# cyberlife-coder/velesdb

Measured on AMD Instinct MI355X. Metric: qps_at_recall10_1Mx768_k10, higher is better.
Workload: dtype f32; 1 GPU; 1000000x768 f32 cosine, k=10, exact distance sweep + fused GPU top-k (BASELINE configs[1]); 1024 queries/step, 1024 queries per corpus pass (sweep_topk_gemm_bf16_pp<dot, WIDE> over normalised bf16 images of rows and queries (cosine; ping-po; rows=1000000, dim=768, k=10, parallelism=replicas x1 (query stream split, no collective)

## Files before the change

velesdb_amd/csrc/g16_protocol.inc:

```
#ifndef VDB_PP_STAMP_AT
#define VDB_PP_STAMP_AT(SLOT) do { } while (0)
#define VDB_G16_OWN_STAMP_STUB 1
#endif
#ifndef VDB_PP_STAMP_COUNT
#define VDB_PP_STAMP_COUNT(SLOT) do { } while (0)
#define VDB_PP_STAMP_ADD(SLOT, N) do { } while (0)
#endif
    VDB_PP_STAMP_AT(16);
    if (hm[0] | hm[1] | hm[2] | hm[3]) VDB_PP_STAMP_COUNT(19);
    VDB_PP_STAMP_ADD(22, __popcll(hm[0]) + __popcll(hm[1]) + __popcll(hm[2]) + __popcll(hm[3]));
    for (;;) {
      ++epoch;
      VDB_PP_STAMP_COUNT(23);
      bool pend = false;
      {
        const uint32_t ln1 = lane_now();
        uint32_t fill = qcnt;
        uint32_t hsz = 64u;
        bool stop = false;
#define VDB_G16_SCAN(T) \
        while (hm[T] && !stop) { \
          if (hsz == 1u && fill + 32u > (uint32_t)QCAP) {  \
            stop = true; \
            break; \
          } \
          const uint32_t hrank = __builtin_amdgcn_mbcnt_hi((uint32_t)(hm[T] >> 32), __builtin_amdgcn_mbcnt_lo((uint32_t)hm[T], 0u)); \
          const bool mine = (((hm[T] >> ln1) & 1ull) != 0) & (hrank < hsz); \
          const uint64_t msk = __ballot(mine); \
          uint32_t nf = fill; \
          const uint32_t hi0 = ((uint32_t)(wr * 128) + 4u * (ln1 >> 4)) | (((uint32_t)(wq * 64 + (T) * 16) + (ln1 & 15u)) << 8); \
_Pragma("unroll") \
          for (int g8 = 0; g8 < 4; g8++) { \
            if (!__ballot(mine & (((gmv[T] >> g8) & 1u) != 0u))) continue;  \
_Pragma("unroll") \
            for (int j8 = 0; j8 < 8; j8++) { \
// ... 20 lines not shown
            if (lanes == 1u) {  \
              stop = true; \
              break; \
            } \
            continue; \
          } \
          fill = nf; \
          hm[T] &= ~msk; \
        }
#define VDB_G16_FINISH(HAVE, RAW, FITS) do { \
          const uint64_t raw_ = (RAW); \
          const uint32_t b = (uint32_t)(raw_ >> 40) & 255u; \
          const float x = __uint_as_float((uint32_t)raw_); \
          const uint32_t rl = (uint32_t)(raw_ >> 32) & 255u; \
          const uint32_t row = rt * BM + rl; \
          float score; \
          if (METRIC == kHamming) {   \
            score = 0.5f * (qn[b] - x); \
          } else if (METRIC == kJaccard) {   \
            const float uni = qn[b] + vns[rl] - x; \
            score = uni == 0.0f ? 1.0f : x / uni; \
          } else { \
            score = halfp ? finish_score_half<METRIC>(x, qn[b], METRIC == kCosine ? vns[rl] : 1.0f) \
                          : finish_score<METRIC>(x, qn[b], METRIC == kCosine ? vns[rl] : 1.0f); \
          } \
           \
          if constexpr (WIDE) score = canon_nan(score); \
          const uint64_t key = make_key<HIB>(score, row); \
          bool take = (HAVE) & (row < a.n_rows) & (key < tauk[b]); \
          if (take && a.alive) take = a.alive[row] != 0;   \
          if constexpr (WIDE) { \
             \
            if (take) { \
              const uint32_t si = atomicAdd(&cnts[b], 1u); \
              if (si < (uint32_t)CAP) { \
                cand[(size_t)b * CAP + si] = key; \
              } else { \
                const uint32_t qg = q0 + b; \
                const uint32_t gi = atomicAdd(&a.wide_cnt[qg], 1u); \
                if (gi < a.wide_cap) a.wide_keys[(size_t)qg * a.wide_cap + gi] = key; \
              } \
            } \
            FITS = true; \
          } else { \
          const uint64_t mt = __ballot(take); \
          FITS = qcnt + (uint32_t)__popcll(mt) <= (uint32_t)QCAP; \
          if (FITS) { \
            if (take) { \
              const uint32_t slot = qcnt + __builtin_amdgcn_mbcnt_hi((uint32_t)(mt >> 32), __builtin_amdgcn_mbcnt_lo((uint32_t)mt, 0u)); \
              wq_keys[slot] = key; \
              wq_qs[slot] = (uint8_t)b; \
            } \
            qcnt += (uint32_t)__popcll(mt); \
          } \
          } \
        } while (0)
#ifndef VDB_G16_NO_DUMP
        if ((uint32_t)__popcll(hm[0]) + (uint32_t)__popcll(hm[1]) + (uint32_t)__popcll(hm[2]) + (uint32_t)__popcll(hm[3]) <= (uint32_t)kG16DumpMaxLanes) {
          bool dump_ok = true;
          if (hm[0] | hm[1] | hm[2] | hm[3]) VDB_PP_STAMP_COUNT(21);
          float* dump = reinterpret_cast<float*>(wq_keys + 8);
#define VDB_G16_DUMP(T) \
          while (hm[T] && dump_ok) { \
            if (qcnt > 8u) { \
              dump_ok = false; \
              break; \
            } \
            VDB_PP_STAMP_COUNT(24);  \
            const uint32_t h0 = (uint32_t)__builtin_ctzll(hm[T]); \
// ... 37 lines not shown
          if (hm[3]) VDB_G16_MASKS(3);
#undef VDB_G16_MASKS
          gm_lazy = false;
        }
        for (;;) {
          VDB_G16_SCAN(0)
          VDB_G16_SCAN(1)
          VDB_G16_SCAN(2)
          VDB_G16_SCAN(3)
          VDB_PP_STAMP_AT(17);
          if (fill > qcnt) {
            const bool have = ln1 < fill - qcnt;
            const uint64_t raw = have ? wq_keys[qcnt + ln1] : 0ull;
            bool fits;
            VDB_G16_FINISH(have, raw, fits);
            (void)fits;
            fill = qcnt;
            VDB_PP_STAMP_AT(18);
          }
          if (!stop) break;
          if (qcnt + 32u > (uint32_t)QCAP) {
            pend = true;
            break;
          }
          stop = false;
        }
#undef VDB_G16_SCAN
#undef VDB_G16_FINISH
      }
      VDB_PP_STAMP_AT(12);
      if constexpr (WIDE) {
        __syncthreads();
        VDB_PP_STAMP_AT(13);
        break;
      }
      if (pend || (last && qcnt)) flags[0] = epoch;
      __syncthreads();
      VDB_PP_STAMP_AT(13);
      if constexpr (!WIDE) {
      if (flags[1] == epoch) {
        compact();
        __syncthreads();
        VDB_PP_STAMP_AT(14);
      }
      }
      bool want = false;
      {
        const uint32_t ln3 = lane_now();
        const uint64_t key = ln3 < qcnt ? wq_keys[ln3] : kKeyInvalid;
        const uint32_t b = ln3 < qcnt ? wq_qs[ln3] : 0u;
        bool full = false;
        if (key != kKeyInvalid && key < tauk[b]) {
          const uint32_t idx = atomicAdd(&cnts[b], 1u);
          if (idx < (uint32_t)CAP) {
            cand[(size_t)b * CAP + idx] = key;
            want = idx >= k;
          } else {
            full = true;
            want = true;
          }
        }
        const uint64_t mf = __ballot(full);
        qcnt = (uint32_t)__popcll(mf);
        if (full) {
          const uint32_t slot = __builtin_amdgcn_mbcnt_hi((uint32_t)(mf >> 32), __builtin_amdgcn_mbcnt_lo((uint32_t)mf, 0u));
          wq_keys[slot] = key;
          wq_qs[slot] = (uint8_t)b;
        }
      }
      if (__ballot(want)) flags[1] = epoch + 1;
      VDB_PP_STAMP_AT(15);
      bool again = flags[0] >= epoch;
      if (last) {
        if (qcnt) flags[2] = epoch;
        __syncthreads();
        again |= flags[2] == epoch;
      }
      if (!again) break;
    }
#ifdef VDB_G16_OWN_STAMP_STUB
#undef VDB_PP_STAMP_AT
#undef VDB_G16_OWN_STAMP_STUB
#endif
```

velesdb_amd/csrc/g16_writeout.inc:

```
  if constexpr (WIDE) {
  __syncthreads();
  uint32_t* wbase = reinterpret_cast<uint32_t*>(qn);
  const uint32_t t_o = (uint32_t)wib * 64u + lane_now();
  if (t_o < nq_t) {
    const uint32_t n = min(cnts[t_o], (uint32_t)CAP);
    wbase[t_o] = n ? atomicAdd(&a.wide_cnt[q0 + t_o], n) : 0u;
  }
  __syncthreads();
  for (uint32_t i = t_o; i < nq_t * (uint32_t)CAP; i += (uint32_t)WAVES * 64u) {
    const uint32_t b = i / (uint32_t)CAP, e = i - b * (uint32_t)CAP;
    const uint32_t pos = wbase[b] + e;
    if (e < cnts[b] && pos < a.wide_cap) a.wide_keys[(size_t)(q0 + b) * a.wide_cap + pos] = cand[i];
  }
  }
  if constexpr (!WIDE) {
  __syncthreads();
  compact();
  __syncthreads();
  const uint32_t lane_o = lane_now();
  for (uint32_t b = wib; b < nq_t; b += WAVES) {
    const uint32_t c = min(cnts[b], k);
    uint64_t* out = a.part_keys + ((size_t)(q0 + b) * a.list_stride + a.list_off + g) * k;
    for (uint32_t e = lane_o; e < k; e += 64) out[e] = e < c ? cand[(size_t)b * CAP + e] : kKeyInvalid;
    if (a.blk_tau && lane_o == 0) a.blk_tau[(size_t)(q0 + b) * a.list_stride + a.list_off + g] = tauk[b];
  }
  }
```

velesdb_amd/csrc/select_stage.hip:

```cpp
#include <algorithm>
#include <array>
#include <cstdio>
#include <cstdlib>
#include <cstring>
#include <string>
#include <vector>

#include "vdb_probe_env.hpp"
#include "vdb_select_stage.hpp"
#include "vdb_wide.hpp"

namespace vdb {

static inline uint32_t opt_max_tile(const vdb_hip_index* ix) { return (uint32_t)opt_value(ix, VDB_OPT_MAX_QUERY_TILE); }
static inline int opt_engine(const vdb_hip_index* ix) { return (int)opt_value(ix, VDB_OPT_SWEEP_ENGINE); }
static inline int opt_selector(const vdb_hip_index* ix) { return (int)opt_value(ix, VDB_OPT_SELECTOR_LEVEL); }
static const bool g_bf16_seed = [] {
  const char* e = probe_env("VELESDB_BF16_SEED");
  return !(e && e[0] == '0');
}();
static const bool g_pool_select = [] {
  const char* e = probe_env("VELESDB_POOL_SELECT");
  return !(e && e[0] == '0');
}();
// ... 786 lines not shown
        mf.skip_cnt = qcount;
        mf.skip_le = kFallbackGatherMax;
      }
      launch_merge(true, mf, nqg, st);
      fin.fb_ids = mf.out_ids;
      fin.fb_scores = mf.out_scores;
      fin.fb_n = mf.out_n;
    }
    if (gather_ok) {
      fin.max_listed = gather_all ? 0u : kFallbackGatherMax;
      fin.g_ids = mg.out_ids;
      fin.g_scores = mg.out_scores;
      fin.g_n = mg.out_n;
    }
    launch_select_finish(fin, st);
  }
  ix->split_flags_off = o_flags;
  ix->split_flags_n = nqg;
  ix->split_flags_stream = st;
  if (ev) (void)hipEventRecord(ev->b, st);
  VDB_HIP(hipGetLastError());
  return VDB_OK;
}


static const bool g_wide_small_k = [] {
  const char* e = probe_env("VELESDB_WIDE_SMALL_K");
  return !(e && e[0] == '0');
}();
static const bool g_wide_fuse = [] {
  const char* e = probe_env("VELESDB_WIDE_FUSE");
  return !(e && e[0] == '0');
}();
int select_level_wide(vdb_hip_index* ix, uint32_t nq_left, uint32_t k, bool sq8) {
  if (opt_selector(ix) < 2 || (!sq8 && opt_engine(ix) != 1) || opt_max_tile(ix) < 128) return 0;
  if (ix->metric != VDB_COSINE && ix->metric != VDB_DOT && (sq8 || ix->metric != VDB_EUCLIDEAN)) return 0;
  if (ix->dim % 64 != 0 || ix->dim < 128 || ix->row_stride != ix->dim) return 0;
  if (k == 0 || k > kWideMaxK || ix->n_rows < kGemmBf16MinRows || ix->n_rows >= 0xFFFFFF00ull) return 0;
  if (k <= kGemmBf16MaxK && (opt_selector(ix) < 3 || !g_wide_small_k)) return 0;
  if (!sq8 && ix->metric != VDB_EUCLIDEAN && sweep_mfma_lds_bytes(1, k, ix->dim) > 160 * 1024) return 0;
  if (!sq8 && ix->metric == VDB_EUCLIDEAN && !l2_gather_fits(ix->dim, k)) return 0;
  if (!select_chunk(nq_left, sq8 ? kSelectMinQueriesSq8 : 0)) return 0;
  if (ix->sel_stats && ix->sel_stats[2] != ix->sel_seq_seen) {
    ix->sel_seq_seen = ix->sel_stats[2];
    if (ix->sel_stats[3] == 4u && (uint64_t)ix->sel_stats[0] * 16 > ix->sel_stats[1]) ix->wide_hold = 64;
  }
  if (ix->wide_hold) {
    ix->wide_hold--;
    return 0;
  }
  return 4;
}

int32_t brute_wide_dev(vdb_hip_index* ix, const float* d_q, uint64_t q_stride, uint32_t nqg, uint32_t k, uint64_t* d_ids, float* d_scores,
                       uint32_t* d_n, hipStream_t st, bool sq8) {
  const bool cosn = !sq8 && cosine_normalised(ix);
  const bool l2 = !sq8 && ix->metric == VDB_EUCLIDEAN;
  const int sel_metric = (cosn || l2) ? VDB_DOT : ix->metric;
  int32_t rc = sq8 ? ensure_sq8_select(ix, st) : (l2 ? ensure_l2_select(ix, st) : (cosn ? ensure_cosn(ix, st) : ensure_sel16(ix, st)));
  if (rc != VDB_OK) return rc;
  const uint32_t dim_a = ix->dim + 64, dim_s = ix->dim + 4;
  const uint16_t* img_rows = sq8 ? ix->sq8_img.as<uint16_t>()
                                 : (l2 ? ix->l2_img.as<uint16_t>() : (cosn ? ix->cosn_img.as<uint16_t>() : ix->rows_bf16.as<uint16_t>()));
  const uint64_t img_stride = l2 ? (uint64_t)dim_a : ((cosn || sq8) ? (uint64_t)ix->dim : ix->bf16_stride);
  const DevBuf& rho_buf = sq8 ? ix->sq8_rho : (l2 ? ix->l2_rho : (cosn ? ix->cosn_rho : ix->bf16_rho));
  const float* sel_norms = sq8 ? ix->sq8_nrm.as<float>() : ix->norms.as<float>();
  DevBuf& list_buf = sq8 ? ix->s_part_cnt : ix->s_fb_keys;
  const uint32_t sel_dim = l2 ? dim_a : ix->dim;
  ix->last_select_level = 4;
  ix->last_kernels |= VDB_KERNEL_SELECT_BF16;
  const uint8_t* alive = ix->any_dead ? ix->alive.as<uint8_t>() : nullptr;
  const uint32_t n = (uint32_t)ix->n_rows, dim = ix->dim;
  static const uint32_t g_small_seed_rows = [] {
    const char* e = probe_env("VELESDB_WIDE_SEED_ROWS");
    const long v = e ? atol(e) : 0;
    return v >= 1024 && v <= (long)kWideSeedRows ? (uint32_t)v / 256u * 256u : kSplitSeedRows;
  }();
  const uint32_t R0 = std::min<uint32_t>(k <= kWideSmallSeedMaxK ? g_small_seed_rows : kWideSeedRows, n), ngrp = (R0 + 15) / 16;
  GemmSchedule sch;
  {
    static const std::array<uint32_t, 3> mult = [] {
      std::array<uint32_t, 3> m{1, 4, 16};
      if (const char* e = probe_env("VELESDB_WIDE_STEPS")) {
        unsigned a = 0, b = 0, c = 0;
        const int got = sscanf(e, "%u,%u,%u", &a, &b, &c);
        m = {got >= 1 ? a : 0u, got >= 2 ? b : 0u, got >= 3 ? c : 0u};
      }
      return m;
    }();
    const uint32_t head[3] = {mult[0], mult[1], mult[2]};
    gemm_schedule(nqg, 0, n, ix->n_cus, head, 0, &sch);
  }
  int g_nqt = 3;
  while (g_nqt > 1 && sweep_mfma_lds_bytes(g_nqt, k, dim) > 160 * 1024) g_nqt--;
  const int g_waves = g_nqt >= 2 ? kMfmaWaves2 : kMfmaWaves1;
  const uint32_t g_B = l2 ? 8u : (uint32_t)g_nqt * 16;
  const uint32_t ntiles16 = (n + 15) / 16;
  const int g_blocks = l2 ? blocks_for(ix, 8, (n + 7) / 8)
                          : (int)std::max<int64_t>(1, std::min<int64_t>(((int64_t)ntiles16 + g_waves - 1) / g_waves, (int64_t)ix->n_cus));
  size_t off = 0;
  auto take = [&](size_t bytes) {
    const size_t o = off;
    off = (off + bytes + 15) & ~(size_t)15;
    return o;
  };
  const size_t o_tau = take((size_t)nqg * 8), o_delta = take((size_t)nqg * 4), o_qn = take((size_t)nqg * 4), o_rho = take((size_t)nqg * 4),
               o_cnt = take((size_t)nqg * 4), o_state = take((size_t)nqg * 4), o_flags = take((size_t)nqg * 4 + 16), o_qmap = take((size_t)nqg * 8),
               o_gid = take((size_t)nqg * k * 8), o_gsc = take((size_t)nqg * k * 4), o_gn = take((size_t)nqg * 4), o_nmax = take(16),
               o_extra = take((size_t)nqg * 4);
  hipError_t e;
  if ((e = ix->s_seed.reserve(off, false, st)) != hipSuccess || (e = list_buf.reserve((size_t)nqg * kWideCap * 8, false, st)) != hipSuccess ||
      (e = ix->s_part_keys.reserve((size_t)nqg * ngrp * 8, false, st)) != hipSuccess ||
      (!sq8 && (e = ix->s_part_cnt.reserve((size_t)nqg * g_blocks * k * 8, false, st)) != hipSuccess) ||
      (e = ix->s_misc.reserve(((size_t)nqg + 256) * img_stride * 2 + (l2 ? (size_t)nqg * dim_s * 4 + 16 : 0), false, st)) != hipSuccess)
    return fail(VDB_ERR_OOM, "wide selection scratch");
  unsigned char* sd = ix->s_seed.as<unsigned char>();
  uint16_t* q16 = ix->s_misc.as<uint16_t>();
  float* qnorms = reinterpret_cast<float*>(sd + o_qn);
  float* rho_q = rho_buf.p ? reinterpret_cast<float*>(sd + o_rho) : nullptr;
  uint32_t* flags = reinterpret_cast<uint32_t*>(sd + o_flags);
  uint32_t* qcount = flags + nqg;
  uint32_t* qmap = reinterpret_cast<uint32_t*>(sd + o_qmap);
  uint32_t* qslot = qmap + nqg;
  uint32_t* norm_max = reinterpret_cast<uint32_t*>(sd + o_nmax);
  EventPair* ev = next_events(ix);
  if (ev) (void)hipEventRecord(ev->a, st);
  if (l2) {
    float* qaug = reinterpret_cast<float*>(ix->s_misc.as<unsigned char>() + ((((size_t)nqg + 256) * img_stride * 2 + 15) & ~(size_t)15));
    launch_l2_augment_queries(d_q, q_stride, q16, dim_a, qaug, dim_s, nqg, dim, st);
    if (rho_q) launch_query_round_error(d_q, q_stride, rho_q, nqg, dim, st);
    PrepArgs pq{};
    pq.rows = d_q;
    pq.norms = qnorms;
    pq.row_stride = q_stride;
    pq.n_rows = nqg;
    pq.dim = dim;
    pq.words = ix->words;
    launch_prep_rows(pq, st);
    VDB_HIP(hipMemsetAsync(flags, 0, (size_t)nqg * 4 + 16, st));
  } else if (cosn) launch_seln_prep_queries(d_q, q_stride, q16, img_stride, qnorms, rho_q, flags, nqg + 4, nqg, dim, st);
  else launch_sel16_prep_queries(d_q, q_stride, q16, img_stride, qnorms, rho_q, flags, nqg + 4, nqg, dim, st);
  if (nqg % 256u) VDB_HIP(hipMemsetAsync(q16 + (size_t)nqg * img_stride, 0, (size_t)256 * img_stride * 2, st));
  if (ix->metric == VDB_DOT || l2) launch_max_norm(sel_norms, n, norm_max, st);
  WideArgs wa{};
  wa.keys = list_buf.as<uint64_t>();
  wa.eps_extra = sq8 ? 1.5e-4f : 0.0f;
  wa.cnt = reinterpret_cast<uint32_t*>(sd + o_cnt);
  wa.state = reinterpret_cast<uint32_t*>(sd + o_state);
  wa.tau = reinterpret_cast<uint64_t*>(sd + o_tau);
  wa.delta = reinterpret_cast<float*>(sd + o_delta);
  wa.qnorms = qnorms;
  wa.rho_q = rho_q;
  wa.rho_max_bits = rho_q ? rho_buf.as<uint32_t>() : nullptr;
  wa.norm_max_bits = norm_max;
  wa.extra = l2 ? reinterpret_cast<float*>(sd + o_extra) : nullptr;
  wa.cap = kWideCap;
  wa.k = k;
  wa.dim = dim;
  launch_seed_scores_bf16(sel_metric, img_rows, img_stride, sel_norms, alive, q16, img_stride, qnorms, ix->s_part_keys.as<uint64_t>(), R0,
                          nqg, sel_dim, st);
  if (l2) launch_wide_seed_l2(wa, ix->s_part_keys.as<uint64_t>(), ngrp, dim_a, nqg, st);
  else launch_wide_seed(ix->metric, wa, ix->s_part_keys.as<uint64_t>(), ngrp, nqg, st);
  for (int j = 0; j < sch.n_launch; j++) {
    EventPair* evs = next_sel_events(ix);
    if (evs) (void)hipEventRecord(evs->a, st);
    e = launch_sweep_gemm_bf16_wide(sel_metric, sch.bp[j], img_rows, img_stride, sel_norms, alive, q16, img_stride, wa.tau, wa.keys, wa.cnt,
                                    wa.cap, sel_dim, nqg, st, qnorms);
    if (evs) (void)hipEventRecord(evs->b, st);
    if (e != hipSuccess) return fail(VDB_ERR_HIP, std::string("wide selection launch: ") + hipGetErrorString(e));
    if (j + 1 < sch.n_launch || l2 || sq8 || !g_wide_fuse) launch_wide_reseed(wa, nqg, st);
  }
  WideOutArgs wo{};
  wo.rows = ix->rows.as<float>();
  wo.norms = ix->norms.as<float>();
  wo.queries = d_q;
  wo.ext_ids = ix->ext_ids.as<uint64_t>();
  wo.out_ids = d_ids;
  wo.out_scores = d_scores;
  wo.out_n = d_n;
  wo.flags = flags;
  wo.qcount = qcount;
  wo.qmap = qmap;
  wo.qslot = qslot;
  wo.row_stride = ix->row_stride;
  wo.q_stride = q_stride;
  wo.dim_pad = (dim + 127) / 128 * 128;
  if (sq8) {
    wo.sq8_codes = ix->sq8_codes.as<uint8_t>();
    wo.sq8_min = ix->sq8_min.as<float>();
    wo.sq8_max = ix->sq8_max.as<float>();
    wo.sq8_nsq = ix->sq8_nsq.as<float>();
    wo.sq8_stride = ix->sq8_stride;
    launch_wide_rerank_sq8(ix->metric, wa, wo, nqg, st);
    SelectFinishArgs fq{};
    fq.flags = flags;
    fq.qcount = qcount;
    fq.qslot = qslot;
    fq.out_ids = d_ids;
    fq.out_scores = d_scores;
    fq.out_n = d_n;
    fq.nq = nqg;
    fq.k = k;
    if (ix->sel_stats) {
// ... 107 lines not shown
```

velesdb_amd/csrc/sweep_gemm_bf16.hip:

```cpp
#include <algorithm>

#include "vdb_probe_env.hpp"
#include "vdb_device.hpp"
#include "vdb_kernels.hpp"

namespace vdb {

typedef float f32x4 __attribute__((ext_vector_type(4)));
typedef __bf16 bf16x8 __attribute__((ext_vector_type(8)));
typedef __attribute__((address_space(3))) void* lds_ptr_t;
typedef __attribute__((address_space(3))) uint32_t lds_u32_t;

constexpr int kG16BM = 256, kG16BN = 256, kG16Waves = 8;
constexpr int kG16Cap = 12;
constexpr int kG16Queue = 39;
#ifndef VDB_G16_DUMP_MAX_LANES
#define VDB_G16_DUMP_MAX_LANES 6
#endif
constexpr int kG16DumpMaxLanes = VDB_G16_DUMP_MAX_LANES;
static_assert(kG16Queue == 39, "g16_protocol.inc keeps two hot lanes' 64 accumulators in queue entries 8 .. 39");
static_assert(kG16Queue <= 64 && kG16Queue >= 32, "the finish pass takes one queue entry per lane; one hot lane's 32 elements fit");
constexpr size_t kOffCand = 131072, kOffTauk = kOffCand + (size_t)kG16BN * kG16Cap * 8, kOffCnts = kOffTauk + kG16BN * 8,
                 kOffQn = kOffCnts + kG16BN * 4, kOffVns = kOffQn + kG16BN * 4, kOffFlags = kOffVns + kG16BM * 4,
                 kOffQueue = kOffFlags + 16,
                 kQueueBytes = 368,
                
                 kG16Lds = kOffQueue + kG16Waves * kQueueBytes;
static_assert(kG16Lds <= 160 * 1024, "LDS budget");
static_assert((size_t)(kG16Queue + 1) * 8 + kG16Queue + 4 <= 364 + 4 && (size_t)(kG16Queue + 1) * 8 + kG16Queue <= 364, "queue layout");

struct Bf16GemmArgs {
  const uint16_t* rows;
  const float* norms;
  const uint8_t* alive;
  const uint16_t* queries;
  const uint64_t* tau0;
  uint64_t* part_keys;
  uint64_t row_stride, q_stride;
  uint32_t n_rows, dim, nq, k;
  uint32_t KT, G, nqt, qper;
  uint32_t row_tile0;
  uint32_t list_stride, list_off;
  const float* qnorms;
  uint64_t* blk_tau;
  const float* qnorms_half;
  unsigned long long* dbg;
  uint64_t* wide_keys;
  uint32_t* wide_cnt;
  uint32_t wide_cap;
};

__device__ __forceinline__ uint32_t lane_now() {
  uint32_t l;
  asm volatile("v_mbcnt_lo_u32_b32 %0, -1, 0\n\tv_mbcnt_hi_u32_b32 %0, -1, %0" : "=v"(l));
  return l;
}

__device__ __forceinline__ void mfma_bf16_inplace(f32x4& c, const f32x4& a, const f32x4& b) {
  asm volatile("v_mfma_f32_16x16x32_bf16 %0, %1, %2, %0" : "+v"(c) : "v"(a), "v"(b));
}
__device__ __forceinline__ void mfma_bf16_first(f32x4& c, const f32x4& a, const f32x4& b) {
  asm volatile("v_mfma_f32_16x16x32_bf16 %0, %1, %2, 0" : "=&v"(c) : "v"(a), "v"(b));
}
__device__ __forceinline__ void mfma_drain() { asm volatile("s_nop 15\n\ts_nop 15" ::: "memory"); }

typedef int i32x4 __attribute__((ext_vector_type(4)));
__device__ __forceinline__ void glds_b128(const i32x4& rsrc, uint32_t voff, uint32_t soff, uint32_t lds_addr) {
  asm volatile("s_mov_b32 m0, %3\n\ts_nop 3\n\tbuffer_load_dwordx4 %0, %1, %2 offen lds"
               :
               : "v"(voff), "s"(rsrc), "s"(soff), "s"(lds_addr)
               : "m0");
}
__device__ __forceinline__ i32x4 make_rsrc(const void* base, uint32_t num_records = 0x7FFFFFFFu) {
  const uint64_t b = reinterpret_cast<uint64_t>(base);
  return i32x4{(int)(uint32_t)b, (int)((uint32_t)(b >> 32) & 0xFFFFu), (int)num_records, 0x00020000};
}
__device__ __forceinline__ i32x4 make_rsrc_uniform(const void* base, uint32_t num_records = 0x7FFFFFFFu) {
  const uint64_t b = reinterpret_cast<uint64_t>(base);
  const uint32_t lo = (uint32_t)__builtin_amdgcn_readfirstlane((int)(uint32_t)b);
  const uint32_t hi = (uint32_t)__builtin_amdgcn_readfirstlane((int)(uint32_t)(b >> 32));
  return i32x4{(int)lo, (int)(hi & 0xFFFFu), __builtin_amdgcn_readfirstlane((int)num_records), 0x00020000};
}
__device__ __forceinline__ uint32_t a_tile_records(uint32_t n_rows, uint32_t rt, uint32_t kt, uint64_t row_stride) {
// ... 241 lines not shown
  static_assert(FP4 == (METRIC == kHamming || METRIC == kJaccard), "the four-bit instance serves the bit metrics, the bf16 instance Cosine / DotProduct");
  constexpr bool HIB = METRIC != kHamming;
  constexpr int BM = kG16BM, BN = kG16BN, WAVES = kG16Waves, CAP = kG16Cap, QCAP = kG16Queue;
  extern __shared__ __attribute__((aligned(16))) unsigned char smem[];
  uint64_t* cand = reinterpret_cast<uint64_t*>(smem + kOffCand);
  uint64_t* tauk = reinterpret_cast<uint64_t*>(smem + kOffTauk);
  uint32_t* cnts = reinterpret_cast<uint32_t*>(smem + kOffCnts);
  float* qn = reinterpret_cast<float*>(smem + kOffQn);
  float* vns = reinterpret_cast<float*>(smem + kOffVns);
  volatile lds_u32_t* flags = (volatile lds_u32_t*)(lds_ptr_t)(smem + kOffFlags);

  const int tid = (int)threadIdx.x;
  const int lane = tid & 63;
  const int wib = __builtin_amdgcn_readfirstlane(tid >> 6);
  const int wr = wib >> 2, wq = wib & 3;
  uint64_t* wq_keys = reinterpret_cast<uint64_t*>(smem + kOffQueue + (size_t)wib * kQueueBytes);
  uint8_t* wq_qs = reinterpret_cast<uint8_t*>(wq_keys + QCAP + 1);

  const uint32_t bid = blockIdx.x;
  const uint32_t xcd = bid & 7u, slot_id = bid >> 3;
  const uint32_t qt = slot_id % a.nqt;
  const uint32_t g = (slot_id / a.nqt) * 8u + xcd;
  const uint32_t q0 = qt * a.qper;
  const uint32_t nq_t = min(a.qper, a.nq - q0);
  const uint32_t k = a.k;
  const uint16_t* queries = a.queries + (size_t)q0 * a.q_stride;

  if (tid < BN) {
    cnts[tid] = 0;
    tauk[tid] = ((uint32_t)tid < nq_t && a.tau0) ? a.tau0[q0 + tid] : kKeyInvalid;
    qn[tid] = 0.0f;
  }
  if (tid < 4) flags[tid] = 0u;
  __syncthreads();
  if (a.qnorms) {
    if ((uint32_t)tid < nq_t) qn[tid] = a.qnorms[q0 + tid];
  } else if (a.qnorms_half) {
    if ((uint32_t)tid < nq_t) qn[tid] = a.qnorms_half[q0 + tid];
  } else {
    for (uint32_t b = wib; b < nq_t; b += WAVES) {
      const uint16_t* qp = queries + (size_t)b * a.q_stride;
      float nacc = 0.0f;
      for (uint32_t c = lane; c * 4 < a.dim; c += 64)
#pragma unroll
        for (int e = 0; e < 4; e++) {
          const uint32_t i = c * 4 + e;
          if (i < a.dim) {
            const float x = F16 ? (float)__builtin_bit_cast(_Float16, qp[i]) : __uint_as_float((uint32_t)qp[i] << 16);
            nacc = __builtin_fmaf(x, x, nacc);
          }
        }
      const float n = sqrtf(butterfly_all(nacc));
      if (lane == 0) qn[b] = n;
    }
  }
  __syncthreads();
  const uint32_t ntiles = (a.n_rows + BM - 1) / BM;
  const uint32_t rt_first = a.row_tile0 + g;
  const uint32_t my_tiles = rt_first < ntiles ? (ntiles - rt_first + a.G - 1) / a.G : 0;
  const uint32_t total = my_tiles * a.KT;

  uint32_t voff_a, voff_b;
  int a_rd0, b_rd0, rd_x;
#define VDB_PP_LANE() do { \
    const uint32_t ln_ = lane_now(); \
    const uint32_t st_row_ = (uint32_t)wib * 8u + (ln_ >> 3); \
// ... 145 lines not shown
    VDB_PP_MFMA(a1v, 4, 2, FIRST); \
    VDB_PP_STAMP_AT(5); \
    pp_barrier(); \
    VDB_PP_STAMP_AT(6); \
     \
     \
    VDB_PP_LPART(if (!(LAST)) VDB_PP_READ_A(a0v, 0, buf ^ 1u), VDB_PP_REQ_A(1, rt2, kt2, buf)); \
    VDB_PP_STAMP_ISSUE(7); \
    pp_wait_dma6(); \
    pp_barrier_reads_done(); \
    VDB_PP_STAMP_AT(4); \
    VDB_PP_MFMA(a1v, 4, 0, FIRST); \
    VDB_PP_STAMP_AT(5); \
    pp_barrier(); \
    VDB_PP_STAMP_AT(6); \
    VDB_PP_NEXT2(); \
    c++; \
  } while (0)

#if VDB_PP_STAMP
  if (st_on) {
    uint64_t t_;
    asm volatile("s_memtime %0\n\ts_waitcnt lgkmcnt(0)" : "=s"(t_)::"memory");
    st_last = (uint32_t)t_;
  }
#endif
  for (uint32_t rt = rt_first; rt < ntiles; rt += a.G) {
    VDB_PP_KTILE(true, false);
    for (uint32_t kt = 1; kt + 1 < a.KT; kt++) VDB_PP_KTILE(false, false);
    VDB_PP_KTILE(false, true);
    const bool more = c < total;
    if (wr == 0) pp_barrier();
    VDB_PP_STAMP_AT(11);
#define VDB_G16_ACC_F(V) (V)
#include "g16_quicktest.inc"
    if constexpr (METRIC == kHamming || METRIC == kJaccard) {
#include "g16_quicktest_bits.inc"
    } else {
#include "g16_quicktest_dense.inc"
    }
    VDB_PP_STAMP_AT(10);
#define VDB_G16_ACC_ELEM(X, A) asm volatile("v_mov_b32 %0, %1" : "=v"(X) : "v"(A))
#include "g16_protocol.inc"
#undef VDB_G16_ACC_ELEM
#undef VDB_G16_ACC_F
    VDB_PP_LANE();
    VDB_PP_READ_A(a0v, 0, c & 1u);
    if (more && wr == 1) pp_barrier();
    VDB_PP_STAMP_AT(8);
  }
#undef VDB_PP_KTILE
#undef VDB_PP_LANE
#undef VDB_PP_NEXT2
#undef VDB_PP_MFMA
#undef VDB_PP_READ_B
#undef VDB_PP_READ_A
#undef VDB_PP_REQ_B
#undef VDB_PP_REQ_A
  asm volatile("s_waitcnt vmcnt(0)" ::: "memory");
#if VDB_PP_STAMP
  if (st_on && lane_now() == 0) {
    st_acc[9] = c;
    unsigned long long* d = a.dbg + (size_t)(wib == 0 ? 0 : 1) * 28;
    for (int i = 0; i < 28; i++) d[i] = st_acc[i];
  }
#endif
#include "g16_writeout.inc"
}
template <int METRIC, bool FP4 = false, bool WIDE = false>
__global__ __launch_bounds__(512, 2) void sweep_topk_gemm_bf16_pp(Bf16GemmArgs a) { gemm16_pp_body<METRIC, FP4, WIDE, false>(a); }
template <int METRIC>
__global__ __launch_bounds__(512, 2) void sweep_topk_gemm_f16_pp(Bf16GemmArgs a) { gemm16_pp_body<METRIC, false, false, true>(a); }

template <bool F16>
__global__ __launch_bounds__(256) void query_norms_bf16_kernel(const uint16_t* q16, uint64_t q_stride, float* out, uint32_t nq, uint32_t dim) {
  const uint32_t lane = threadIdx.x & 63u, b = blockIdx.x * 4u + (threadIdx.x >> 6);
// ... 102 lines not shown
  hipLaunchKernelGGL((sweep_topk_gemm_bf16_pp<METRIC, false, true>), dim3(blocks), dim3(512), kG16Lds, st, a);
  return hipGetLastError();
}

template <int METRIC>
static hipError_t launch_g16_fp4(const Bf16GemmArgs& a, int blocks, hipStream_t st) {
  static bool done = false;
  if (!done) {
    hipError_t e = hipFuncSetAttribute(reinterpret_cast<const void*>(&sweep_topk_gemm_bf16_pp<METRIC, true>),
                                       hipFuncAttributeMaxDynamicSharedMemorySize, 160 * 1024);
    if (e != hipSuccess) return e;
    done = true;
  }
  hipLaunchKernelGGL((sweep_topk_gemm_bf16_pp<METRIC, true>), dim3(blocks), dim3(512), kG16Lds, st, a);
  return hipGetLastError();
}

template <int METRIC, bool SPLIT>
static hipError_t launch_g16(const Bf16GemmArgs& a, int blocks, hipStream_t st) {
  static bool done = false;
  if (!done) {
    hipError_t e = hipFuncSetAttribute(reinterpret_cast<const void*>(&sweep_topk_gemm_bf16_glds<METRIC, SPLIT>),
                                       hipFuncAttributeMaxDynamicSharedMemorySize, 160 * 1024);
    if (e != hipSuccess) return e;
    done = true;
  }
  hipLaunchKernelGGL((sweep_topk_gemm_bf16_glds<METRIC, SPLIT>), dim3(blocks), dim3(512), kG16Lds, st, a);
  return hipGetLastError();
}

hipError_t launch_sweep_gemm_bf16_wide(int metric, const Bf16GemmPlan& p, const uint16_t* rows16, uint64_t row_stride, const float* norms,
                                       const uint8_t* alive, const uint16_t* queries16, uint64_t q_stride, const uint64_t* tau0,
                                       uint64_t* wide_keys, uint32_t* wide_cnt, uint32_t wide_cap, uint32_t dim, uint32_t nq, hipStream_t st,
                                       const float* qnorms) {
  Bf16GemmArgs a{};
  a.rows = rows16;
  a.norms = norms;
  a.alive = alive;
  a.queries = queries16;
  a.tau0 = tau0;
  a.row_stride = row_stride;
  a.q_stride = q_stride;
  a.n_rows = p.row_hi;
  a.row_tile0 = p.row_lo / kG16BM;
  a.dim = dim;
  a.nq = nq;
  a.k = kGemmBf16MaxK;
  a.KT = dim / 64;
  a.G = p.G;
  a.nqt = p.nqt;
  a.qper = p.qper;
  a.qnorms = qnorms;
  a.wide_keys = wide_keys;
  a.wide_cnt = wide_cnt;
  a.wide_cap = wide_cap;
#if VDB_PP_STAMP
  a.dbg = pp_stamp_dbg();
#endif
  return metric == kCosine ? launch_g16_wide<kCosine>(a, p.blocks, st) : launch_g16_wide<kDot>(a, p.blocks, st);
}

hipError_t launch_sweep_gemm_bf16_glds(int metric, const Bf16GemmPlan& p, const uint16_t* rows16, uint64_t row_stride,
                                       const float* norms, const uint8_t* alive, const uint16_t* queries16, uint64_t q_stride,
                                       const uint64_t* tau0, uint64_t* part_keys, uint32_t list_stride, uint32_t list_off,
                                       uint32_t dim, uint32_t nq, uint32_t k, hipStream_t st, bool split, const float* qnorms,
                                       uint64_t* blk_tau, const float* qnorms_half, bool f16) {
  Bf16GemmArgs a{};
  a.rows = rows16;
// ... 38 lines not shown
```

velesdb_amd/csrc/sweep_wide.hip:

```cpp
#include <algorithm>

#include "vdb_device.hpp"
#include "vdb_kernels.hpp"
#include "vdb_wide.hpp"
#include "vdb_block_select.hpp"

namespace vdb {

__device__ __forceinline__ float wide_eps(uint32_t dim, const float* rho_q, const uint32_t* rho_max_bits, uint32_t q, float extra = 0.0f) {
  const float acc = 16.0f * (float)dim * 5.9604645e-8f;
  if (!rho_q || !rho_max_bits) return 2.0f * 3.90625e-3f * 1.002f + 1.6e-5f + acc + extra;
  const float rm = __uint_as_float(*rho_max_bits), rq = rho_q[q];
  return (rm + rq + 3.0f * rm * rq) * 1.002f + acc + 4e-6f + extra;
}

__device__ __forceinline__ uint64_t wide_tau_key(float s_k, float delta, bool* ok, float extra = 0.0f) {
  const float lowered = s_k - 2.0f * delta * 1.01f - extra - fabsf(s_k) * 1e-6f;
  *ok = lowered == lowered && fabsf(lowered) < 3.0e38f;
  return make_key<true>(lowered, 0u);
}
__device__ __forceinline__ uint64_t wide_tau_closed() { return make_key<true>(3.0e38f, 0u); }

template <int METRIC>
__global__ __launch_bounds__(256) void wide_seed_kernel(WideArgs a, const uint64_t* seed_keys, uint32_t ngrp) {
  __shared__ uint32_t hist[256];
  __shared__ uint32_t ctl[2];
  const uint32_t q = blockIdx.x, tid = threadIdx.x;
  constexpr int NPT = kWideSeedGroups / 256;
  uint64_t keys[NPT];
  uint32_t mine = 0;
#pragma unroll
  for (int j = 0; j < NPT; j++) {
    const uint32_t i = tid + 256u * (uint32_t)j;
    keys[j] = i < ngrp ? seed_keys[(size_t)q * ngrp + i] : kKeyInvalid;
    mine += keys[j] != kKeyInvalid ? 1u : 0u;
  }
  const float eps = wide_eps(a.dim, a.rho_q, a.rho_max_bits, q, a.eps_extra);
  const float d = METRIC == kCosine ? eps * 1.001f + 4e-7f : eps * 1.001f * a.qnorms[q] * __uint_as_float(*a.norm_max_bits) + 1e-30f;
  __shared__ uint32_t total;
  if (tid == 0) total = 0;
  __syncthreads();
  if (mine) atomicAdd(&total, mine);
  __syncthreads();
  const uint32_t valid = total;
  bool ok = valid >= a.k && d == d;
  uint64_t tau = wide_tau_closed();
  if (ok) {
    __shared__ uint64_t s256[256];
    const uint32_t hi = ngrp <= 256 ? block_kth_hi_256(keys[0], a.k, s256, ctl) : block_kth_hi<NPT>(keys, a.k, hist, ctl);
    tau = wide_tau_key(key_score<true>((uint64_t)hi << 32), d, &ok);
    if (!ok) tau = wide_tau_closed();
  }
  if (tid == 0) {
    a.delta[q] = d;
    a.tau[q] = tau;
    a.cnt[q] = 0;
    a.state[q] = ok ? 0u : kWideGivenUp;
  }
}

template <int NPT>
__device__ int wide_next_tau(const WideArgs& a, uint32_t raw, const uint64_t (&keys)[NPT], float delta, float extra, uint64_t old, uint32_t* hist,
                             uint32_t* ctl, uint64_t* s256, uint64_t* tau_out) {
  if (raw > a.cap) return 2;
  if (raw < a.k) return 0;
  const uint32_t hi = raw <= 256 ? block_kth_hi_256(keys[0], a.k, s256, ctl, (raw + 7u) & ~7u) : block_kth_hi<NPT>(keys, a.k, hist, ctl);
  bool ok;
  uint64_t tau = wide_tau_key(key_score<true>((uint64_t)hi << 32), delta, &ok, extra);
  if (!ok) return 2;
  if (tau > old) tau = old;
  *tau_out = tau;
  return 1;
}

__global__ __launch_bounds__(256) void wide_reseed_kernel(WideArgs a) {
  __shared__ uint32_t hist[256];
  __shared__ uint32_t ctl[2];
  __shared__ uint32_t wsum[4];
  __shared__ uint64_t s256[256];
  const uint32_t q = blockIdx.x, tid = threadIdx.x;
  const uint32_t state = a.state[q], raw = a.cnt[q];
  const float delta = a.delta[q], extra = a.extra ? a.extra[q] : 0.0f;
  const uint64_t old = a.tau[q];
  if (state & kWideGivenUp) return;
// ... 494 lines not shown
```

velesdb_amd/csrc/vdb_wide.hpp:

```cpp
#pragma once
#include <hip/hip_runtime.h>
#include <stdint.h>

#include "vdb_gemm_schedule.hpp"

namespace vdb {

constexpr uint32_t kWideMaxK = 128;
constexpr uint32_t kWideCap = 4096;
constexpr uint32_t kWidePoolMax = 1024;
constexpr uint32_t kWideSeedRows = 16384;
constexpr uint32_t kWideSeedGroups = kWideSeedRows / 16;
constexpr uint32_t kWideSmallSeedMaxK = 32;
constexpr uint32_t kWideGivenUp = 1u;

struct WideArgs {
  uint64_t* keys;
  uint32_t* cnt;
  uint32_t* state;
  uint64_t* tau;
  float* delta;
  const float* qnorms;
  const float* rho_q;
  const uint32_t* rho_max_bits;
  const uint32_t* norm_max_bits;
  float* extra;
  uint32_t cap, k, dim;
  float eps_extra;
};
struct WideOutArgs {
  const float* rows;
  const float* norms;
  const float* queries;
  const uint64_t* ext_ids;
  uint64_t* out_ids;
  float* out_scores;
  uint32_t* out_n;
  uint32_t* flags;
  uint32_t* qcount;
  uint32_t* qmap;
  uint32_t* qslot;
  uint64_t row_stride, q_stride;
  uint32_t dim_pad;
  const uint8_t* sq8_codes;
  const float* sq8_min;
  const float* sq8_max;
  const float* sq8_nsq;
  uint64_t sq8_stride;
  unsigned long long* stamps;
};

void launch_wide_seed(int metric, const WideArgs& a, const uint64_t* seed_keys, uint32_t ngrp, uint32_t nq, hipStream_t st);
void launch_wide_reseed(const WideArgs& a, uint32_t nq, hipStream_t st);
void launch_wide_rerank(int metric, const WideArgs& a, const WideOutArgs& o, uint32_t nq, bool fuse_final_reseed, hipStream_t st);
void launch_wide_seed_l2(const WideArgs& a, const uint64_t* seed_keys, uint32_t ngrp, uint32_t dim_a, uint32_t nq, hipStream_t st);
void launch_wide_rerank_l2(const WideArgs& a, const WideOutArgs& o, uint32_t nq, hipStream_t st);
void launch_wide_rerank_sq8(int metric, const WideArgs& a, const WideOutArgs& o, uint32_t nq, hipStream_t st);
hipError_t launch_sweep_gemm_bf16_wide(int metric, const Bf16GemmPlan& p, const uint16_t* rows16, uint64_t row_stride, const float* norms,
                                       const uint8_t* alive, const uint16_t* queries16, uint64_t q_stride, const uint64_t* tau0,
                                       uint64_t* wide_keys, uint32_t* wide_cnt, uint32_t wide_cap, uint32_t dim, uint32_t nq, hipStream_t st,
                                       const float* qnorms);

}
```

Baseline: 756,200 queries/s.

## Tighten wide top-k threshold in-kernel with a per-query score ladder histogram

During the wide bf16 sweep, each accepted candidate bumps a global per-query counter in one of 16 score bands above the seed's k-th score. Each block reads these counts at start and after each ping-pong tile and lowers its local tau to the highest band that already holds k hits. With this in-kernel tightening in place, the stepped multi-launch schedule and the reseed kernels between launches are dropped in favour of large single launches. The aim is to filter more rows and cut launch and reseed overhead, at the cost of extra global atomics per candidate, giving up one stash slot per query, and some prefetch register pressure.

```diff
diff --git a/velesdb_amd/csrc/g16_protocol.inc b/velesdb_amd/csrc/g16_protocol.inc
--- a/velesdb_amd/csrc/g16_protocol.inc
+++ b/velesdb_amd/csrc/g16_protocol.inc
@@ -1,6 +1,12 @@
 #ifndef VDB_PP_STAMP_AT
 #define VDB_PP_STAMP_AT(SLOT) do { } while (0)
 #define VDB_G16_OWN_STAMP_STUB 1
+#endif
+#ifndef VDB_G16_STASH_CAP
+#define VDB_G16_STASH_CAP ((uint32_t)CAP)
+#define VDB_G16_LADDER_COUNT(B, SCORE) do { } while (0)
+#define VDB_G16_LADDER_REFRESH() do { } while (0)
+#define VDB_G16_OWN_LADDER_STUB 1
 #endif
 #ifndef VDB_PP_STAMP_COUNT
 #define VDB_PP_STAMP_COUNT(SLOT) do { } while (0)
@@ -87,9 +93,11 @@
           if constexpr (WIDE) { \
              \
             if (take) { \
+              VDB_G16_LADDER_COUNT(b, score); \
+              const uint32_t scap_ = VDB_G16_STASH_CAP; \
               const uint32_t si = atomicAdd(&cnts[b], 1u); \
-              if (si < (uint32_t)CAP) { \
-                cand[(size_t)b * CAP + si] = key; \
+              if (si < scap_) { \
+                cand[(size_t)b * scap_ + si] = key; \
               } else { \
                 const uint32_t qg = q0 + b; \
                 const uint32_t gi = atomicAdd(&a.wide_cnt[qg], 1u); \
@@ -193,6 +201,7 @@
       if constexpr (WIDE) {
         __syncthreads();
         VDB_PP_STAMP_AT(13);
+        VDB_G16_LADDER_REFRESH();
         break;
       }
       if (pend || (last && qcnt)) flags[0] = epoch;
@@ -239,6 +248,12 @@
       }
       if (!again) break;
     }
+#ifdef VDB_G16_OWN_LADDER_STUB
+#undef VDB_G16_STASH_CAP
+#undef VDB_G16_LADDER_COUNT
+#undef VDB_G16_LADDER_REFRESH
+#undef VDB_G16_OWN_LADDER_STUB
+#endif
 #ifdef VDB_G16_OWN_STAMP_STUB
 #undef VDB_PP_STAMP_AT
 #undef VDB_G16_OWN_STAMP_STUB
diff --git a/velesdb_amd/csrc/g16_writeout.inc b/velesdb_amd/csrc/g16_writeout.inc
--- a/velesdb_amd/csrc/g16_writeout.inc
+++ b/velesdb_amd/csrc/g16_writeout.inc
@@ -1,14 +1,15 @@
   if constexpr (WIDE) {
   __syncthreads();
+  const uint32_t scap = a.lad ? (uint32_t)CAP - 1u : (uint32_t)CAP;
   uint32_t* wbase = reinterpret_cast<uint32_t*>(qn);
   const uint32_t t_o = (uint32_t)wib * 64u + lane_now();
   if (t_o < nq_t) {
-    const uint32_t n = min(cnts[t_o], (uint32_t)CAP);
+    const uint32_t n = min(cnts[t_o], scap);
     wbase[t_o] = n ? atomicAdd(&a.wide_cnt[q0 + t_o], n) : 0u;
   }
   __syncthreads();
-  for (uint32_t i = t_o; i < nq_t * (uint32_t)CAP; i += (uint32_t)WAVES * 64u) {
-    const uint32_t b = i / (uint32_t)CAP, e = i - b * (uint32_t)CAP;
+  for (uint32_t i = t_o; i < nq_t * scap; i += (uint32_t)WAVES * 64u) {
+    const uint32_t b = i / scap, e = i - b * scap;
     const uint32_t pos = wbase[b] + e;
     if (e < cnts[b] && pos < a.wide_cap) a.wide_keys[(size_t)(q0 + b) * a.wide_cap + pos] = cand[i];
   }
diff --git a/velesdb_amd/csrc/select_stage.hip b/velesdb_amd/csrc/select_stage.hip
--- a/velesdb_amd/csrc/select_stage.hip
+++ b/velesdb_amd/csrc/select_stage.hip
@@ -842,6 +842,11 @@
   const char* e = probe_env("VELESDB_WIDE_FUSE");
   return !(e && e[0] == '0');
 }();
+static const bool g_wide_ladder = [] {
+  const char* e = probe_env("VELESDB_WIDE_LADDER");
+  return !(e && e[0] == '0');
+}();
+constexpr uint32_t kWideLadderLaunchRows = 2u << 20;
 int select_level_wide(vdb_hip_index* ix, uint32_t nq_left, uint32_t k, bool sq8) {
   if (opt_selector(ix) < 2 || (!sq8 && opt_engine(ix) != 1) || opt_max_tile(ix) < 128) return 0;
   if (ix->metric != VDB_COSINE && ix->metric != VDB_DOT && (sq8 || ix->metric != VDB_EUCLIDEAN)) return 0;
@@ -887,8 +892,12 @@
     return v >= 1024 && v <= (long)kWideSeedRows ? (uint32_t)v / 256u * 256u : kSplitSeedRows;
   }();
   const uint32_t R0 = std::min<uint32_t>(k <= kWideSmallSeedMaxK ? g_small_seed_rows : kWideSeedRows, n), ngrp = (R0 + 15) / 16;
+  const bool ladder = !l2 && !sq8 && k <= kWideSmallSeedMaxK && g_wide_ladder;
   GemmSchedule sch;
-  {
+  if (ladder) {
+    const uint32_t head[3] = {0, 0, 0};
+    gemm_schedule(nqg, 0, n, ix->n_cus, head, kWideLadderLaunchRows, &sch);
+  } else {
     static const std::array<uint32_t, 3> mult = [] {
       std::array<uint32_t, 3> m{1, 4, 16};
       if (const char* e = probe_env("VELESDB_WIDE_STEPS")) {
@@ -917,7 +926,8 @@
   const size_t o_tau = take((size_t)nqg * 8), o_delta = take((size_t)nqg * 4), o_qn = take((size_t)nqg * 4), o_rho = take((size_t)nqg * 4),
                o_cnt = take((size_t)nqg * 4), o_state = take((size_t)nqg * 4), o_flags = take((size_t)nqg * 4 + 16), o_qmap = take((size_t)nqg * 8),
                o_gid = take((size_t)nqg * k * 8), o_gsc = take((size_t)nqg * k * 4), o_gn = take((size_t)nqg * 4), o_nmax = take(16),
-               o_extra = take((size_t)nqg * 4);
+               o_extra = take((size_t)nqg * 4), o_ladpar = take((size_t)nqg * sizeof(WideLadderPar)),
+               o_lad = take((size_t)nqg * kWideLadderLevels * 4 + 64);
   hipError_t e;
   if ((e = ix->s_seed.reserve(off, false, st)) != hipSuccess || (e = list_buf.reserve((size_t)nqg * kWideCap * 8, false, st)) != hipSuccess ||
       (e = ix->s_part_keys.reserve((size_t)nqg * ngrp * 8, false, st)) != hipSuccess ||
@@ -967,6 +977,10 @@
   wa.cap = kWideCap;
   wa.k = k;
   wa.dim = dim;
+  if (ladder) {
+    wa.lad = reinterpret_cast<uint32_t*>((reinterpret_cast<uintptr_t>(sd + o_lad) + 63) & ~(uintptr_t)63);
+    wa.lad_par = reinterpret_cast<WideLadderPar*>(sd + o_ladpar);
+  }
   launch_seed_scores_bf16(sel_metric, img_rows, img_stride, sel_norms, alive, q16, img_stride, qnorms, ix->s_part_keys.as<uint64_t>(), R0,
                           nqg, sel_dim, st);
   if (l2) launch_wide_seed_l2(wa, ix->s_part_keys.as<uint64_t>(), ngrp, dim_a, nqg, st);
@@ -975,10 +989,10 @@
     EventPair* evs = next_sel_events(ix);
     if (evs) (void)hipEventRecord(evs->a, st);
     e = launch_sweep_gemm_bf16_wide(sel_metric, sch.bp[j], img_rows, img_stride, sel_norms, alive, q16, img_stride, wa.tau, wa.keys, wa.cnt,
-                                    wa.cap, sel_dim, nqg, st, qnorms);
+                                    wa.cap, sel_dim, nqg, st, qnorms, wa.lad, wa.lad_par, wa.delta, k);
     if (evs) (void)hipEventRecord(evs->b, st);
     if (e != hipSuccess) return fail(VDB_ERR_HIP, std::string("wide selection launch: ") + hipGetErrorString(e));
-    if (j + 1 < sch.n_launch || l2 || sq8 || !g_wide_fuse) launch_wide_reseed(wa, nqg, st);
+    if (j + 1 < sch.n_launch ? !ladder : (l2 || sq8 || !g_wide_fuse)) launch_wide_reseed(wa, nqg, st);
   }
   WideOutArgs wo{};
   wo.rows = ix->rows.as<float>();
diff --git a/velesdb_amd/csrc/sweep_gemm_bf16.hip b/velesdb_amd/csrc/sweep_gemm_bf16.hip
--- a/velesdb_amd/csrc/sweep_gemm_bf16.hip
+++ b/velesdb_amd/csrc/sweep_gemm_bf16.hip
@@ -3,6 +3,7 @@
 #include "vdb_probe_env.hpp"
 #include "vdb_device.hpp"
 #include "vdb_kernels.hpp"
+#include "vdb_wide.hpp"
 
 namespace vdb {
 
@@ -48,7 +49,31 @@
   uint64_t* wide_keys;
   uint32_t* wide_cnt;
   uint32_t wide_cap;
+  uint32_t* lad;
+  const WideLadderPar* lad_par;
+  const float* lad_delta;
+  uint32_t lad_k;
 };
+constexpr int kG16LadCap = kG16Cap - 1;
+constexpr size_t kOffLadPar = kOffCand + (size_t)kG16BN * kG16LadCap * 8;
+static_assert(kOffLadPar + (size_t)kG16BN * sizeof(WideLadderPar) == kOffTauk && sizeof(WideLadderPar) == 8, "the ladder parameters take the twelfth slot row");
+typedef __attribute__((address_space(1))) uint32_t glb_u32_t;
+typedef uint32_t u32x4 __attribute__((ext_vector_type(4)));
+template <int OFF>
+__device__ __forceinline__ void ladder_load_b128(u32x4& dst, const void* p) {
+  asm volatile("global_load_dwordx4 %0, %1, off offset:%2 sc1" : "=v"(dst) : "v"(p), "n"(OFF));
+}
+__device__ __forceinline__ void ladder_load_b32(uint32_t& dst, const void* p) {
+  asm volatile("global_load_dword %0, %1, off sc1" : "=v"(dst) : "v"(p));
+}
+__device__ __forceinline__ void ladder_loads_wait(u32x4& c0, u32x4& c1, u32x4& c2, u32x4& c3, uint32_t& x, uint32_t& y) {
+  asm volatile("s_waitcnt vmcnt(0)" : "+v"(c0), "+v"(c1), "+v"(c2), "+v"(c3), "+v"(x), "+v"(y)::"memory");
+}
+__device__ __forceinline__ uint64_t ladder_refresh_regs(uint64_t old, const u32x4& c0, const u32x4& c1, const u32x4& c2, const u32x4& c3, uint32_t k,
+                                                        WideLadderPar lp, float delta, uint32_t list_cnt, uint32_t list_cap) {
+  const uint32_t cnt[kWideLadderLevels] = {c0[0], c0[1], c0[2], c0[3], c1[0], c1[1], c1[2], c1[3], c2[0], c2[1], c2[2], c2[3], c3[0], c3[1], c3[2], c3[3]};
+  return wide_ladder_refresh(old, cnt, k, lp, delta, list_cnt, list_cap);
+}
 
 __device__ __forceinline__ uint32_t lane_now() {
   uint32_t l;
@@ -356,6 +381,28 @@
     qn[tid] = 0.0f;
   }
   if (tid < 4) flags[tid] = 0u;
+  WideLadderPar* ladp = reinterpret_cast<WideLadderPar*>(smem + kOffLadPar);
+  if constexpr (WIDE) {
+    if (a.lad && tid < BN) {
+      const bool inq = (uint32_t)tid < nq_t;
+      const WideLadderPar lp = inq ? a.lad_par[q0 + tid] : WideLadderPar{__uint_as_float(0x7F800000u), 0.0f};
+      ladp[tid] = lp;
+      if (inq) {
+        const uint32_t qg = q0 + (uint32_t)tid;
+        const unsigned char* lq = reinterpret_cast<const unsigned char*>(a.lad + (size_t)qg * kWideLadderLevels);
+        u32x4 c0, c1, c2, c3;
+        uint32_t dl, gc;
+        ladder_load_b128<0>(c0, lq);
+        ladder_load_b128<16>(c1, lq);
+        ladder_load_b128<32>(c2, lq);
+        ladder_load_b128<48>(c3, lq);
+        ladder_load_b32(dl, a.lad_delta + qg);
+        ladder_load_b32(gc, a.wide_cnt + qg);
+        ladder_loads_wait(c0, c1, c2, c3, dl, gc);
+        tauk[tid] = ladder_refresh_regs(tauk[tid], c0, c1, c2, c3, a.lad_k, lp, __uint_as_float(dl), gc, a.wide_cap);
+      }
+    }
+  }
   __syncthreads();
   if (a.qnorms) {
     if ((uint32_t)tid < nq_t) qn[tid] = a.qnorms[q0 + tid];
@@ -567,6 +614,23 @@
     const bool more = c < total;
     if (wr == 0) pp_barrier();
     VDB_PP_STAMP_AT(11);
+    u32x4 ldc0 = {0u, 0u, 0u, 0u}, ldc1 = ldc0, ldc2 = ldc0, ldc3 = ldc0;
+    uint32_t ld_dl = 0u, ld_gc = 0u;
+    bool lad_on = false;
+    if constexpr (WIDE) {
+      lad_on = a.lad != nullptr;
+      if (lad_on && wr == 0) {
+        const uint32_t qg = q0 + min((uint32_t)wib * 64u + lane_now(), nq_t - 1u);
+        const unsigned char* lq = reinterpret_cast<const unsigned char*>(a.lad + (size_t)qg * kWideLadderLevels);
+        ladder_load_b128<0>(ldc0, lq);
+        ladder_load_b128<16>(ldc1, lq);
+        ladder_load_b128<32>(ldc2, lq);
+        ladder_load_b128<48>(ldc3, lq);
+        ladder_load_b32(ld_dl, a.lad_delta + qg);
+        ladder_load_b32(ld_gc, a.wide_cnt + qg);
+      }
+    }
+    (void)lad_on;
 #define VDB_G16_ACC_F(V) (V)
 #include "g16_quicktest.inc"
     if constexpr (METRIC == kHamming || METRIC == kJaccard) {
@@ -576,7 +640,25 @@
     }
     VDB_PP_STAMP_AT(10);
 #define VDB_G16_ACC_ELEM(X, A) asm volatile("v_mov_b32 %0, %1" : "=v"(X) : "v"(A))
+#define VDB_G16_STASH_CAP (lad_on ? (uint32_t)kG16LadCap : (uint32_t)CAP)
+#define VDB_G16_LADDER_COUNT(B, SCORE) do { \
+      if (lad_on) { \
+        const WideLadderPar lp_ = ladp[B]; \
+        const uint32_t lv_ = wide_ladder_level((SCORE), lp_.base, lp_.step); \
+        if (lv_) (void)__hip_atomic_fetch_add((glb_u32_t*)a.lad + ((size_t)(q0 + (B)) * kWideLadderLevels + (lv_ - 1u)), 1u, __ATOMIC_RELAXED, __HIP_MEMORY_SCOPE_AGENT); \
+      } \
+    } while (0)
+#define VDB_G16_LADDER_REFRESH() do { \
+      if (lad_on && wr == 0) { \
+        ladder_loads_wait(ldc0, ldc1, ldc2, ldc3, ld_dl, ld_gc); \
+        const uint32_t b_ = (uint32_t)wib * 64u + lane_now(); \
+        if (b_ < nq_t) tauk[b_] = ladder_refresh_regs(tauk[b_], ldc0, ldc1, ldc2, ldc3, a.lad_k, ladp[b_], __uint_as_float(ld_dl), ld_gc, a.wide_cap); \
+      } \
+    } while (0)
 #include "g16_protocol.inc"
+#undef VDB_G16_LADDER_REFRESH
+#undef VDB_G16_LADDER_COUNT
+#undef VDB_G16_STASH_CAP
 #undef VDB_G16_ACC_ELEM
 #undef VDB_G16_ACC_F
     VDB_PP_LANE();
@@ -745,8 +827,14 @@
 hipError_t launch_sweep_gemm_bf16_wide(int metric, const Bf16GemmPlan& p, const uint16_t* rows16, uint64_t row_stride, const float* norms,
                                        const uint8_t* alive, const uint16_t* queries16, uint64_t q_stride, const uint64_t* tau0,
                                        uint64_t* wide_keys, uint32_t* wide_cnt, uint32_t wide_cap, uint32_t dim, uint32_t nq, hipStream_t st,
-                                       const float* qnorms) {
+                                       const float* qnorms, uint32_t* lad, const WideLadderPar* lad_par, const float* lad_delta, uint32_t lad_k) {
   Bf16GemmArgs a{};
+  if (lad && lad_par && lad_delta && lad_k) {
+    a.lad = lad;
+    a.lad_par = lad_par;
+    a.lad_delta = lad_delta;
+    a.lad_k = lad_k;
+  }
   a.rows = rows16;
   a.norms = norms;
   a.alive = alive;
diff --git a/velesdb_amd/csrc/sweep_wide.hip b/velesdb_amd/csrc/sweep_wide.hip
--- a/velesdb_amd/csrc/sweep_wide.hip
+++ b/velesdb_amd/csrc/sweep_wide.hip
@@ -14,12 +14,6 @@
   return (rm + rq + 3.0f * rm * rq) * 1.002f + acc + 4e-6f + extra;
 }
 
-__device__ __forceinline__ uint64_t wide_tau_key(float s_k, float delta, bool* ok, float extra = 0.0f) {
-  const float lowered = s_k - 2.0f * delta * 1.01f - extra - fabsf(s_k) * 1e-6f;
-  *ok = lowered == lowered && fabsf(lowered) < 3.0e38f;
-  return make_key<true>(lowered, 0u);
-}
-__device__ __forceinline__ uint64_t wide_tau_closed() { return make_key<true>(3.0e38f, 0u); }
 
 template <int METRIC>
 __global__ __launch_bounds__(256) void wide_seed_kernel(WideArgs a, const uint64_t* seed_keys, uint32_t ngrp) {
@@ -45,11 +39,36 @@
   const uint32_t valid = total;
   bool ok = valid >= a.k && d == d;
   uint64_t tau = wide_tau_closed();
+  uint32_t kth_hi = 0;
   if (ok) {
     __shared__ uint64_t s256[256];
     const uint32_t hi = ngrp <= 256 ? block_kth_hi_256(keys[0], a.k, s256, ctl) : block_kth_hi<NPT>(keys, a.k, hist, ctl);
+    kth_hi = hi;
     tau = wide_tau_key(key_score<true>((uint64_t)hi << 32), d, &ok);
     if (!ok) tau = wide_tau_closed();
+  }
+  if (a.lad) {
+    __shared__ uint32_t wbest[4];
+    uint32_t best = 0xFFFFFFFFu;
+#pragma unroll
+    for (int j = 0; j < NPT; j++) best = min(best, (uint32_t)(keys[j] >> 32));
+#pragma unroll
+    for (int o = 32; o >= 1; o >>= 1) best = min(best, (uint32_t)__shfl_xor((int)best, o, 64));
+    if ((tid & 63u) == 0) wbest[tid >> 6] = best;
+    __syncthreads();
+    if (tid < kWideLadderLevels) a.lad[(size_t)q * kWideLadderLevels + tid] = 0u;
+    if (tid == 0) {
+      WideLadderPar lp{__uint_as_float(0x7F800000u), 0.0f};
+      if (ok) {
+        const float sk = key_score<true>((uint64_t)kth_hi << 32);
+        const float sb = key_score<true>((uint64_t)min(min(wbest[0], wbest[1]), min(wbest[2], wbest[3])) << 32);
+        float step = fmaxf(3.0f * (sb - sk) / (float)kWideLadderLevels, d);
+        if (!(step >= 0.0f) || !(step <= 3.4028235e38f)) step = 0.0f;
+        lp.base = sk;
+        lp.step = step;
+      }
+      a.lad_par[q] = lp;
+    }
   }
   if (tid == 0) {
     a.delta[q] = d;
diff --git a/velesdb_amd/csrc/vdb_wide.hpp b/velesdb_amd/csrc/vdb_wide.hpp
--- a/velesdb_amd/csrc/vdb_wide.hpp
+++ b/velesdb_amd/csrc/vdb_wide.hpp
@@ -1,10 +1,69 @@
 #pragma once
+#include <math.h>
+#include <stdint.h>
+#if defined(__HIPCC__)
 #include <hip/hip_runtime.h>
-#include <stdint.h>
+#define VDB_WIDE_HD __host__ __device__ __forceinline__
+#else
+#define VDB_WIDE_HD inline
+#endif
 
 #include "vdb_gemm_schedule.hpp"
 
 namespace vdb {
+
+constexpr uint32_t kWideLadderLevels = 16;
+struct WideLadderPar {
+  float base, step;
+};
+VDB_WIDE_HD uint32_t wide_f2u(float f) { return __builtin_bit_cast(uint32_t, f); }
+VDB_WIDE_HD float wide_ladder_threshold(float base, float step, uint32_t j) { return __builtin_fmaf((float)j, step, base); }
+VDB_WIDE_HD uint32_t wide_ladder_level(float s, float base, float step) {
+  if (!(fabsf(s) <= 3.4028235e38f) || !(step >= 0.0f) || !(step <= 3.4028235e38f)) return 0u;
+  const float e = (s - base) / step;
+  uint32_t j = e >= 1.0f ? (e < (float)kWideLadderLevels ? (uint32_t)e : kWideLadderLevels) : 0u;
+  if (j < kWideLadderLevels && s >= wide_ladder_threshold(base, step, j + 1u)) j++;
+  if (j && !(s >= wide_ladder_threshold(base, step, j))) j--;
+  if (j && !(s >= wide_ladder_threshold(base, step, j))) j = 0u;
+  return j;
+}
+VDB_WIDE_HD uint32_t wide_ladder_pick(const uint32_t (&cnt)[kWideLadderLevels], uint32_t k) {
+  uint32_t sum = 0, js = 0;
+#if defined(__clang__)
+#pragma unroll
+#endif
+  for (uint32_t j = kWideLadderLevels; j >= 1u; j--) {
+    const uint32_t c = cnt[j - 1u];
+    sum = sum + c < sum ? 0xFFFFFFFFu : sum + c;
+    if (js == 0u && sum >= k) js = j;
+  }
+  return k ? js : 0u;
+}
+VDB_WIDE_HD uint64_t wide_key_of_score(float score) {
+  const uint32_t b = wide_f2u(score);
+  const uint32_t asc = b ^ ((b >> 31) ? 0xFFFFFFFFu : 0x80000000u);
+  return (uint64_t)(~asc) << 32;
+}
+VDB_WIDE_HD uint64_t wide_tau_key(float s_k, float delta, bool* ok, float extra = 0.0f) {
+  const float lowered = s_k - 2.0f * delta * 1.01f - extra - fabsf(s_k) * 1e-6f;
+  *ok = lowered == lowered && fabsf(lowered) < 3.0e38f;
+  return wide_key_of_score(lowered);
+}
+VDB_WIDE_HD uint64_t wide_tau_closed() { return wide_key_of_score(3.0e38f); }
+VDB_WIDE_HD uint64_t wide_ladder_refresh(uint64_t old, const uint32_t (&cnt)[kWideLadderLevels], uint32_t k, WideLadderPar p, float delta,
+                                         uint32_t list_cnt, uint32_t list_cap) {
+  uint64_t t = old;
+  const uint32_t js = wide_ladder_pick(cnt, k);
+  if (js && p.step >= 0.0f && p.step <= 3.4028235e38f) {
+    bool ok;
+    const uint64_t key = wide_tau_key(wide_ladder_threshold(p.base, p.step, js), delta, &ok);
+    if (ok && key < t) t = key;
+  }
+  if (list_cnt > list_cap && wide_tau_closed() < t) t = wide_tau_closed();
+  return t;
+}
+
+#if defined(__HIPCC__)
 
 constexpr uint32_t kWideMaxK = 128;
 constexpr uint32_t kWideCap = 4096;
@@ -26,6 +85,8 @@
   const uint32_t* norm_max_bits;
   float* extra;
   uint32_t cap, k, dim;
+  uint32_t* lad;
+  WideLadderPar* lad_par;
   float eps_extra;
 };
 struct WideOutArgs {
@@ -59,6 +120,8 @@
 hipError_t launch_sweep_gemm_bf16_wide(int metric, const Bf16GemmPlan& p, const uint16_t* rows16, uint64_t row_stride, const float* norms,
                                        const uint8_t* alive, const uint16_t* queries16, uint64_t q_stride, const uint64_t* tau0,
                                        uint64_t* wide_keys, uint32_t* wide_cnt, uint32_t wide_cap, uint32_t dim, uint32_t nq, hipStream_t st,
-                                       const float* qnorms);
+                                       const float* qnorms, uint32_t* lad = nullptr, const WideLadderPar* lad_par = nullptr,
+                                       const float* lad_delta = nullptr, uint32_t lad_k = 0);
+#endif
 
 }
```

After: 729,500 queries/s. 3.5% lower.
